# pierrebarbera/epa-ng

Measured on AMD Instinct MI355X. Metric: query placements/sec (whole node), 512-tip GTR+G4 DNA ref, preplace+thorough, higher is better.
Workload: dtype f64; 1 GPU; cfg2: 512-tip DNA GTR+G4 ref, W=1500, 150 bp reads, dyn-heur 0.99999, preplace+thorough; branches=1021, parallelism=query-shard x1 (weak)

## Files before the change

epa_ng_amd/csrc/epa_dev.hip:

```cpp
#include "epa_dev_internal.hpp"

#include <math.h>
#include <string.h>

#include <algorithm>
#include <numeric>
#include <atomic>
#include <thread>

static thread_local std::string g_create_err;

int epa_fail(epa_ctx* ctx, int code, const std::string& msg) {
  if (ctx) ctx->err = msg; else g_create_err = msg;
  return code;
}

namespace {
__global__ void __launch_bounds__(256) k_zero(uint4* __restrict__ a, size_t na, uint4* __restrict__ b, size_t nb) {
  const size_t stride = (size_t)gridDim.x * 256, i0 = (size_t)blockIdx.x * 256 + threadIdx.x;
  const uint4 z = make_uint4(0u, 0u, 0u, 0u);
  for (size_t i = i0; i < na; i += stride) a[i] = z;
  for (size_t i = i0; i < nb; i += stride) b[i] = z;
}
}
// ... 422 lines not shown
    if (code[t] != EPA_OK) { if (bad_query) *bad_query = bad[t]; return code[t]; }
  return EPA_OK;
}

extern "C" int epa_encode_queries(uint32_t states, uint32_t sites, uint32_t Q,
                                  const char* const* seqs, int premasking, int aa_x_as_n,
                                  uint8_t* codes, uint32_t* win_begin, uint32_t* win_span,
                                  uint32_t* bad_query) {
  return encode_impl(states, sites, Q, seqs, premasking, aa_x_as_n, false, 0, codes, win_begin, win_span,
                     bad_query);
}

extern "C" int epa_encode_queries_compact(uint32_t states, uint32_t sites, uint32_t Q,
                                          const char* const* seqs, int premasking, int aa_x_as_n,
                                          uint32_t stride, uint8_t* codes, uint32_t* win_begin,
                                          uint32_t* win_span, uint32_t* bad_query) {
  if (stride && !codes) return EPA_ERR_INVALID_ARG;
  return encode_impl(states, sites, Q, seqs, premasking, aa_x_as_n, true, stride, codes, win_begin,
                     win_span, bad_query);
}

extern "C" int epa_dev_device_count(void) {
  int n = 0;
  if (hipGetDeviceCount(&n) != hipSuccess) { (void)hipGetLastError(); return 0; }
  return n;
}

extern "C" const char* epa_dev_last_error(const epa_ctx* ctx) {
  return ctx ? ctx->err.c_str() : g_create_err.c_str();
}

extern "C" int epa_dev_set_query_layout(epa_ctx* ctx, uint32_t code_stride) {
  if (!ctx) return EPA_ERR_INVALID_ARG;
  ctx->code_stride = code_stride;
  return EPA_OK;
}

extern "C" int epa_dev_set_option(epa_ctx* ctx, const char* key, int value) {
  if (!ctx || !key) return EPA_ERR_INVALID_ARG;
  if (strcmp(key, "lookup_block") == 0) {
    if (!ctx->lookup_blocks) return epa_fail(ctx, EPA_ERR_INVALID_ARG, "set_option: lookup_block needs a context in the blocked lookup layout");
    if (value <= 0 || (value & 63)) return epa_fail(ctx, EPA_ERR_INVALID_ARG, "set_option: lookup_block must be a positive multiple of 64");
    for (void* p : ctx->blk_buf)
      if (p) return epa_fail(ctx, EPA_ERR_INVALID_ARG, "set_option: lookup_block must be set before the first preplacement");
    ctx->lookup_block = (uint32_t)value;
    return EPA_OK;
  }
  struct Entry { const char* name; int EpaOptions::*field; };
  static const Entry table[] = {
      {"thorough_generic", &EpaOptions::thorough_generic}, {"preplace_generic", &EpaOptions::preplace_generic},
      {"select_full_rows", &EpaOptions::select_full_rows}, {"select_sort", &EpaOptions::select_sort},
      {"queued_thorough", &EpaOptions::queued_thorough},   {"xcd_balance", &EpaOptions::xcd_balance},
      {"aa_valu", &EpaOptions::aa_valu},                   {"timers", &EpaOptions::timers},
      {"newton_lds", &EpaOptions::newton_lds}};
  for (const Entry& e : table)
    if (strcmp(key, e.name) == 0) {
      ctx->opt.*e.field = value;
      ctx->generic_thorough = ctx->generic_native || ctx->opt.thorough_generic != 0;
      return EPA_OK;
    }
  return epa_fail(ctx, EPA_ERR_INVALID_ARG, std::string("set_option: unknown key '") + key + "'");
}

extern "C" int epa_dev_set_heuristic(epa_ctx* ctx, int mode, double param) {
  if (!ctx) return EPA_ERR_INVALID_ARG;
  if (mode < EPA_HEUR_DYNAMIC || mode > EPA_HEUR_BASEBALL)
    return epa_fail(ctx, EPA_ERR_INVALID_ARG, "set_heuristic: unknown mode");
  if (mode == EPA_HEUR_FIXED && !(param >= 0.0 && param <= 1.0))
    return epa_fail(ctx, EPA_ERR_INVALID_ARG, "set_heuristic: the fraction must lie in [0, 1]");
  ctx->heur_mode = mode;
  ctx->heur_param = param;
  return EPA_OK;
}

extern "C" int epa_dev_set_query_packing(epa_ctx* ctx, int bits) {
  if (!ctx) return EPA_ERR_INVALID_ARG;
  if (bits != 8 && bits != 4) return epa_fail(ctx, EPA_ERR_INVALID_ARG, "set_query_packing: 8 or 4 bits per code");
  if (bits == 4 && ctx->s != 4)
    return epa_fail(ctx, EPA_ERR_UNSUPPORTED, "set_query_packing: the 4-bit format holds nucleotide codes only");
  ctx->code_packed4 = bits == 4;
  return EPA_OK;
}

extern "C" int epa_pack_codes_4bit(const uint8_t* codes, uint32_t Q, uint32_t stride, uint8_t* packed) {
  if (!codes || !packed) return EPA_ERR_INVALID_ARG;
  const size_t ps = ((size_t)stride + 1) / 2;
  const unsigned cap = g_encode_threads.load(std::memory_order_relaxed);
  const unsigned hw = cap ? cap : std::max(1u, std::thread::hardware_concurrency());
  const unsigned nt = (unsigned)std::min<uint64_t>(std::min(hw, 32u), std::max<uint64_t>(1, (uint64_t)Q * stride >> 20));
  std::vector<int> bad(nt, 0);
  auto work = [&](unsigned t) {
    const uint32_t q0 = (uint32_t)((uint64_t)Q * t / nt), q1 = (uint32_t)((uint64_t)Q * (t + 1) / nt);
    unsigned over = 0;
    for (uint32_t q = q0; q < q1; ++q) {
      const uint8_t* r = codes + (size_t)q * stride;
      uint8_t* o = packed + (size_t)q * ps;
      for (uint32_t p = 0; p < stride / 2; ++p) {
        const uint8_t hi = r[2 * p], lo = r[2 * p + 1];
        over |= hi | lo;
        o[p] = (uint8_t)((hi << 4) | lo);
      }
      if (stride & 1) { const uint8_t hi = r[stride - 1]; over |= hi; o[ps - 1] = (uint8_t)(hi << 4); }
    }
    bad[t] = over > 15;
  };
  if (nt == 1) work(0);
  else {
// ... 1958 lines not shown
```

epa_ng_amd/csrc/epa_dev_internal.hpp:

```cpp
#pragma once

#include <hip/hip_runtime.h>
#include <stdint.h>

#include <string>
#include <vector>

#include "epa_dev.h"

#define EPA_MAX_STATES 20
#define EPA_MAX_CATS 16
#define EPA_MAX_COLS 24
#define EPA_GRID_Y 65535u

struct ModelDNA {
  double U[16];
  double Ui[16];
  double lam[4];
  double rate[16];
  double w[16];
  double pi[4];
  int ng;
};

// ... 58 lines not shown
  size_t d_unpacked_sz = 0;
  size_t codes_bytes = 0;
  uint32_t Q = 0, stride = 0;
  bool packed4 = false;
  epa_pair* d_pairs = nullptr;
  epa_result* d_res = nullptr;
  size_t cap = 0;
  void* h_out = nullptr;
  size_t h_out_sz = 0;
  unsigned long long* h_stats = nullptr;
  unsigned long long* d_stats = nullptr;
  hipEvent_t ev_up = nullptr, ev_done = nullptr, ev_down = nullptr, ev_base = nullptr;
  hipStream_t stream = nullptr;
  const epa_pair* out_pairs = nullptr;
  const epa_result* out_res = nullptr;
  uint64_t n = 0;
  int state = 0;
  SelectPending sel;
  uint32_t* h_sel = nullptr;
  const uint8_t* l_codes = nullptr;
  const uint32_t *l_begin = nullptr, *l_span = nullptr;
  epa_pair* l_pairs = nullptr;
  epa_result* l_res = nullptr;
  uint32_t l_max_span = 0, l_flags = 0;
  int leader = -1;
  int g_index = 0;
  int g_n = 0;
  int g_left = 0;
  int g_slots[8] = {};
  uint32_t g_qoff[9] = {};
  uint32_t own_Q = 0;
  const uint8_t* own_x_codes = nullptr;
  const uint32_t *own_x_begin = nullptr, *own_x_span = nullptr;
  void* d_merge = nullptr;
  size_t d_merge_sz = 0;
  epa_pair* d_gpairs = nullptr;
  epa_result* d_gres = nullptr;
  size_t g_cap = 0;
  uint32_t* d_goff = nullptr;
  uint32_t* h_goff = nullptr;
};
constexpr int EPA_MAX_GROUP = 8;

struct EpaOptions {
  int thorough_generic = 0;
  int preplace_generic = 0;
  int select_full_rows = 0;
  int select_sort = 0;
  int queued_thorough = 0;
  int xcd_balance = 1;
  int aa_valu = 0;
  int timers = 1;
  int newton_lds = 0;
};

struct epa_ctx {
  int device = 0;
  EpaOptions opt;
  int n_cu = 256;
  hipStream_t stream = nullptr;
  std::string err;

  int s = 0, c = 0, ncols = 0;
  int c_in = 0;
  uint32_t W = 0, B = 0;
  ModelDev hmodel;
  ModelDev* dmodel = nullptr;
  ModelDNA dna;
  bool dna_zero0 = false;
  bool rate_scalers = false;
  bool generic_thorough = false;
  bool generic_native = false;
  BloConsts blo;
  int aa_x_as_n = 0;
  uint32_t code_stride = 0;

  double* refT = nullptr;
  uint32_t* scSum = nullptr;
  double* blen = nullptr;
  double* lookup = nullptr;
  double* refI = nullptr;
  uint8_t* resc0 = nullptr;
  double* cinv = nullptr;
  double inv_w0 = 0.0;
  double* lookup2 = nullptr;
  bool lookup_built = false;
  bool lookup_blocks = false;
  uint32_t lookup_block = 1024;
  std::vector<double> h_blen;

  static constexpr int N_SCRATCH = 18;
  static constexpr int N_SLOTS = 24;
  static constexpr int N_BANKS = 1 + N_SLOTS;
  int bank = 0;
  void* scratch[N_BANKS * N_SCRATCH] = {};
  size_t scratch_sz[N_BANKS * N_SCRATCH] = {};

  uint32_t* d_status = nullptr;
  uint32_t select_cap = 64;
  uint32_t* th_ctr = nullptr;
  uint32_t lnl_pitch = 0;
  unsigned long long* segmax = nullptr;
  uint32_t segp = 0;
  size_t segmax_zero_bytes = 0;
  bool code_packed4 = false;
  int heur_mode = 0;
// ... 107 lines not shown
```

epa_ng_amd/csrc/thorough_dna.hip:

```cpp
#include "epa_dev_internal.hpp"
#include "wave_util.hpp"

#include <cstring>
#include <rocprim/device/device_radix_sort.hpp>

using epa_radix_cfg = rocprim::radix_sort_config<rocprim::default_config, rocprim::default_config,
                                                 rocprim::default_config, 0>;

#include <algorithm>
#include <vector>
#include <cstdio>
#include <type_traits>
#include <cstdlib>

namespace {


struct ThArgs {
  ModelDNA m;
  BloConsts blo;
  const double* refT;
  const double* refI;
  const uint8_t* resc0;
  const double* cinv;
  double inv_w0;
  const uint32_t* scSum;
  const double* blen;
  const double* qt;
  const epa_pair* pairs;
  const uint32_t* order;
  const uint8_t* codes;
  uint32_t cstride, crel;
  const uint32_t* win_begin;
  const uint32_t* win_span;
  epa_result* out;
  unsigned long long* stats;
  uint32_t* qctr;
  double* sscratch;
  uint64_t n_pairs;
  uint32_t W;
  uint32_t Wpad;
  const uint32_t* spec;
  uint32_t spec_cls, spec_max;
  uint32_t xcum[9];
  uint32_t xstamp;
};

using namespace epa_wave;

__device__ __forceinline__ uint32_t zero_after(double v) {
  uint32_t z;
  asm volatile("v_mov_b32 %0, 0" : "=v"(z) : "v"(__double2loint(v)));
  return z;
}

using KArgs = const __attribute__((address_space(4))) ThArgs*;
__device__ __forceinline__ KArgs kargs_fresh() {
  KArgs p = (KArgs)__builtin_amdgcn_kernarg_segment_ptr();
  asm volatile("" : "+s"(p));
  return p;
}
struct PhaseModel {
  double U[16], Ui[16], w[4];
  __device__ __forceinline__ void load(uint32_t grp) {
    KArgs p = kargs_fresh();
#pragma unroll
    for (int i = 0; i < 16; ++i) { U[i] = p->m.U[i]; Ui[i] = p->m.Ui[i]; }
#pragma unroll
    for (int i = 0; i < 4; ++i) w[i] = p->m.w[grp * 4 + i];
  }
};

struct LaneConst {
  double lr;
  double cN;
  double w;
  int slot;
  int npos;
  const double* e2t;
  double lrn;
  double cn[3];
};

template <int N, class F>
__device__ __forceinline__ void static_for(F&& f) {
  if constexpr (N > 0) {
    static_for<N - 1>(f);
    f(std::integral_constant<int, N - 1>{});
  }
}
constexpr int dpp_pos(int k, int x) { return (k >> 1) * 8 + (k & 1) * 3 + x - 1; }
template <int N>
__device__ __forceinline__ void fmac_bcast(double& acc, double t, double s) {
  asm("v_fmac_f64_dpp %0, %1, %2 row_newbcast:%3 row_mask:0xf bank_mask:0xf" : "+v"(acc) : "v"(t), "v"(s), "i"(N));
}
__device__ __forceinline__ void dpp_ready(double& a, double& b, double& c) {
  asm("s_nop 1" : "+v"(a), "+v"(b), "+v"(c));
}
// ... 442 lines not shown
#pragma unroll
  for (int ch = 0; ch < NCH; ++ch) {
    double l0 = lsite[ch];
    bool mine = st.valid[ch];
    if (TAILH && ch == NCH - 1) mine = mine && lane < 32;
    if (!mine) l0 = 1.0;
    const int sc = mine ? (int)(st.sc[ch] + st.resc[ch]) : 0;
    mant *= __builtin_amdgcn_frexp_mant(l0);
    ex += __builtin_amdgcn_frexp_exp(l0) - 256 * sc;
    if ((ch & 7) == 7) {
      ex += __builtin_amdgcn_frexp_exp(mant);
      mant = __builtin_amdgcn_frexp_mant(mant);
    }
  }
  double v = wave_sum(log(mant) + (double)ex * 0.6931471805599453094), z = 0.0;
  cb.sum2(v, z, lane);
  return v;
}

template <int NCH, bool ZERO0, int NW, bool TAILH = false, int NG = 1, bool TDPP = false>
__device__ __forceinline__ double newton(const SiteState<NCH>& st, double* tab, int lane,
                                         const LaneConst& lc, Comb<NW, NG>& cb, double x1, double xguess,
                                         double x2, double tol, int max_iters, uint32_t& evals) {
  double rts = xguess, f, df, xl, xh, dx;
  if (rts < x1) rts = x1;
  if (rts > x2) rts = x2;
  derivatives<NCH, ZERO0, NW, TAILH, NG, TDPP>(st, tab, lane, lc, cb, rts, f, df);
  ++evals;
  if (!isfinite(f) || !isfinite(df)) return NAN;
  if (df >= 0.0 && fabs(f) < tol) return rts;
  if (f < 0.0) { xl = rts; xh = x2; } else { xh = rts; xl = x1; }
  for (int i = 1; i <= max_iters; ++i) {
    if (df <= 0.0 || (((rts - xh) * df - f) * ((rts - xl) * df - f) >= 0.0)) {
      dx = 0.5 * (xh - xl);
      rts = xl + dx;
      if (xl == rts) return rts;
    } else {
      dx = f / df;
      const double temp = rts;
      rts -= dx;
      if (temp == rts) return rts;
    }
    if (fabs(dx) < tol || i == max_iters) return rts;
    if (rts < x1) rts = x1;
    derivatives<NCH, ZERO0, NW, TAILH, NG, TDPP>(st, tab, lane, lc, cb, rts, f, df);
    ++evals;
    if (!isfinite(f) || !isfinite(df)) return NAN;
    if (df > 0.0 && fabs(f) < tol) return rts;
    if (f < 0.0) xl = rts; else xh = rts;
  }
  return NAN;
}

template <int NCH, bool ZERO0, bool INV, int NW, bool LOCAL, bool TAILH = false, int NG = 1, bool TDPP = false>
__device__ __forceinline__ void process_pair(const ThArgs& a, const uint64_t pidx, const int lane,
                                             double* tab, const double* qts, double* qa, const LaneConst& lc,
                                             Comb<NW, NG>& cb, uint32_t (&wstat)[3]) {
  static_assert(NG == 1 || NW == 1, "category groups and site blocks do not combine");
  const uint32_t site0 = NW > 1 ? (uint32_t)cb.wv * NCH * 64 : 0u;
  const uint32_t grp = NG > 1 ? (uint32_t)cb.wv : 0u;
  const uint64_t pid = a.order ? a.order[pidx] : pidx;
  const epa_pair pr = a.pairs[pid];
  const uint32_t b = (uint32_t)__builtin_amdgcn_readfirstlane((int)pr.branch_id);
  const uint32_t q = (uint32_t)__builtin_amdgcn_readfirstlane((int)pr.seq_id);
  const uint32_t begin = (uint32_t)__builtin_amdgcn_readfirstlane((int)a.win_begin[q]);
  const uint32_t n = (uint32_t)__builtin_amdgcn_readfirstlane((int)a.win_span[q]);
  const size_t cW = a.W;
  const char* ref = reinterpret_cast<const char*>(a.refT + ((size_t)(2 * b) * NG + grp) * 16 * cW + begin);
  const uint32_t W8 = a.W * 8u;
  const uint32_t* scp = a.scSum + (size_t)b * cW + begin;
  const uint8_t* qc = a.codes + (size_t)q * a.cstride + (a.crel ? 0u : begin);
  const double orig = a.blen[b];

  SiteState<NCH> st;
  const uint32_t half = TAILH ? (uint32_t)lane >> 5 : 0u;
  const uint32_t hoff = half * 8u * W8;
  double* const tabh = tab + (half << 3);
  auto lane_site = [&](int ch) -> uint32_t {
    return site0 + ch * 64 + ((TAILH && ch == NCH - 1) ? (uint32_t)lane & 31u : (uint32_t)lane);
  };
#pragma unroll
  for (int ch = 0; ch < NCH; ++ch) {
    const uint32_t s = lane_site(ch);
    st.valid[ch] = (NW == 1 && ch < NCH - 1) ? true : s < n;
    const uint32_t sc = st.valid[ch] ? s : 0;
    st.sc[ch] = scp[sc];
    st.code[ch] = qc[sc];
    st.resc[ch] = 0;
  }

  double tp = a.blo.pendant_default, td = orig * 0.5, tx = orig * 0.5;
  uint32_t evals = 0, rounds = 0, reverted = 0;
  uint32_t chain = 0;

  auto cinv_of = [&](int ch) -> double {
    const uint32_t s = st.valid[ch] ? lane_site(ch) : 0;
    const double v = a.cinv[begin + s] * a.inv_w0;
    if (NG > 1 && grp != 0) return 0.0;
    return (TAILH && ch == NCH - 1 && half) ? 0.0 : v;
  };
  const char* refi_s = reinterpret_cast<const char*>(a.refI + ((size_t)b * NG + grp) * 16 * cW + begin);
  auto stream_phase = [&](auto mode_c) {
    constexpr int MODE = decltype(mode_c)::value;
    constexpr int DEPTH = TH_STREAM_DEPTH;
    constexpr int NKL = TAILH ? 2 : 4;
    constexpr int NS = 4 * (NCH - 1) + NKL;
    constexpr int R = DEPTH + 1;
    PhaseModel pm;
    pm.load(grp);
    uint32_t W8p = W8;
    asm volatile("" : "+s"(W8p));
    double An[R][4], Bn[R][4];
    uint32_t soff[NCH], sidx[NCH];
#pragma unroll
    for (int ch = 0; ch < NCH; ++ch) {
      sidx[ch] = st.valid[ch] ? lane_site(ch) : 0;
      soff[ch] = sidx[ch] * 8u + ((TAILH && ch == NCH - 1) ? hoff : 0u);
    }
    uint32_t tok = chain;
    if constexpr (MODE == 1 || MODE == 3) {
      const int kq = lane & 3;
      const double* qv = qts + (lane >> 2) * 4;
      const double* e0 = tab + kq * 4;
      double av[4];
#pragma unroll
      for (int x = 0; x < 4; ++x) av[x] = qv[x] * e0[x];
      double* dst = qa + (lane >> 2) * QA_STRIDE + kq * 4;
#pragma unroll
      for (int i = 0; i < 4; ++i) {
        double v = pm.U[i * 4] * av[0];
#pragma unroll
        for (int x = 1; x < 4; ++x) v = fma(pm.U[i * 4 + x], av[x], v);
        dst[i] = v;
      }
      __builtin_amdgcn_fence(__ATOMIC_RELEASE, "wavefront");
      __builtin_amdgcn_wave_barrier();
      __builtin_amdgcn_fence(__ATOMIC_ACQUIRE, "wavefront");
    }
    auto issue = [&](int stp, uint32_t tk) {
      const int ch = stp >> 2, k = stp & 3, sl = stp % R;
      const uint32_t s0 = soff[ch] + tk;
#pragma unroll
      for (int x = 0; x < 4; ++x) {
        if (MODE == 2) An[sl][x] = *reinterpret_cast<const double*>(refi_s + (s0 + (uint32_t)(k * 4 + x) * W8p));
        else {
          An[sl][x] = *reinterpret_cast<const double*>(ref + (s0 + (uint32_t)(16 * NG + k * 4 + x) * W8p));
          Bn[sl][x] = *reinterpret_cast<const double*>(ref + (s0 + (uint32_t)(k * 4 + x) * W8p));
        }
      }
    };
#pragma unroll
    for (int p = 0; p < DEPTH; ++p)
      if (p < NS) issue(p, tok);
    int mx = 0;
    double qf[4];
#pragma unroll
    for (int stp = 0; stp < NS; ++stp) {
      const int ch = stp >> 2, k = stp & 3, sl = stp % R;
      const bool halfc = TAILH && ch == NCH - 1;
      const int NK = halfc ? 2 : 4;
      const double* tb = halfc ? tabh : tab;
      if (k == 0) {
        const double* qv = qts + st.code[ch] * 4;
        qf[0] = qv[0]; qf[1] = qv[1]; qf[2] = qv[2]; qf[3] = qv[3];
      }
      if (stp + DEPTH < NS) issue(stp + DEPTH, tok);
      asm volatile("" ::: "memory");
      double It[4];
      if (MODE == 2) {
#pragma unroll
        for (int x = 0; x < 4; ++x) It[x] = An[sl][x];
      } else if (MODE == 0) {
        cat_inner(pm, An[sl], tb + k * 4 + 2 * tok, Bn[sl], tb + 16 + k * 4 + 2 * tok, It, mx);
      } else {
        const double* ap = qa + st.code[ch] * QA_STRIDE + ((halfc ? (int)half * 2 : 0) + k) * 4 + 2 * tok;
        double Ap[4];
        lds_pair(ap, Ap[0], Ap[1]); lds_pair(ap + 2, Ap[2], Ap[3]);
        cat_inner_pre(pm, Ap, MODE == 1 ? Bn[sl] : An[sl], tb + 16 + k * 4 + 2 * tok, It, mx);
      }
#pragma unroll
      for (int x = 0; x < 4; ++x)
        st.S[ch][k * 4 + x] = It[x] * ((MODE == 0 || MODE == 2) ? qf[x] : (MODE == 1 ? An[sl][x] : Bn[sl][x]));
      tok = zero_after(st.S[ch][k * 4 + 3]);
      if (k == NK - 1) {
        if (MODE == 2) {
          st.resc[ch] = (a.resc0 + (size_t)b * cW + begin)[sidx[ch]];
        } else {
          int mxs = mx;
          if (halfc) {
            const auto sw = __builtin_amdgcn_permlane32_swap(mx, mx, false, false);
            mxs = max((int)sw[0], (int)sw[1]);
          }
          if constexpr (NG > 1) {
            double mv[1] = {(double)mxs};
            cb.template groups<1, true>(mv, lane);
            mxs = (int)mv[0];
          }
          const uint32_t resc = (mxs < 0x2ff00000) ? 1u : 0u;
          if (__builtin_amdgcn_ballot_w64(resc != 0) != 0) {
            const double mult = resc ? 0x1p+256 : 1.0;
#pragma unroll
            for (int i = 0; i < 16; ++i)
              if (i < NK * 4) st.S[ch][i] *= mult;
          }
          if (MODE == 0) st.resc[ch] = resc;
          mx = 0;
        }
        if constexpr (INV) st.S[ch][0] += cinv_of(ch);
        if constexpr (ZERO0) {
          if (halfc) st.S[ch][0] = fma(half ? pm.w[3] : pm.w[1], st.S[ch][4], (half ? pm.w[2] : pm.w[0]) * st.S[ch][0]);
          else st.S[ch][0] = fma(pm.w[3], st.S[ch][12], fma(pm.w[2], st.S[ch][8], fma(pm.w[1], st.S[ch][4], pm.w[0] * st.S[ch][0])));
        }
        tok = zero_after(st.S[ch][halfc ? 7 : 15]);
      }
    }
    chain = tok;
  };
  auto product_phase = [&](auto mode_c) { stream_phase(mode_c); };
  auto window_score = [&]() -> double {
    double ew[16];
#pragma unroll
    for (int i = 0; i < 8; ++i) lds_pair(tab + 32 + 2 * i, ew[2 * i], ew[2 * i + 1]);
    return window_lnl<NCH, ZERO0, NW, TAILH, NG>(st, ew, cb, lane, tab);
  };
  auto score = [&](double td_, double tx_, double tp_) -> double {
    const double tl = lc.slot == 0 ? td_ : (lc.slot == 1 ? tx_ : tp_);
    table_publish(tab, lane, TH_EXP(lc.lr * tl) * (lc.slot == 2 ? lc.w : 1.0));
    product_phase(std::integral_constant<int, 0>{});
    return window_score();
  };
  auto side_sumtable = [&](double tp_, double tother_, auto toward_prox) {
    constexpr bool TOWARD_PROX = decltype(toward_prox)::value;
    table_publish(tab, lane, TH_EXP(lc.lr * (lc.slot == 0 ? tp_ : tother_)));
    product_phase(std::integral_constant<int, TOWARD_PROX ? 3 : 1>{});
  };
  auto distal_sumtable = [&](double tp_, double tx_) { side_sumtable(tp_, tx_, std::false_type{}); };

  auto score_first = [&](double tp_) -> double {
    table_publish(tab, lane, TH_EXP(lc.lr * tp_) * (lc.slot == 2 ? lc.w : 1.0));
    stream_phase(std::integral_constant<int, 2>{});
    return window_score();
  };

  double loglikelihood = a.refI ? -score_first(tp) : -score(td, tx, tp);

  uint32_t smoothings = a.blo.max_rounds;
  if constexpr (LOCAL) {
    const double xmin = a.blo.min_branch, xmax = a.blo.max_branch, xtol = xmin / 10.0;
    auto solve = [&](double cur) -> double {
      double g = cur;
      if (g < xmin || g > xmax) g = a.blo.default_branch;
      const double r = newton<NCH, ZERO0, NW, TAILH, NG, TDPP>(st, tab, lane, lc, cb, xmin, g, xmax, xtol, (int)a.blo.max_newton, evals);
      chain = zero_after(r);
      return (isfinite(r) && fabs(cur - r) > 1e-10) ? r : cur;
    };
    while (smoothings) {
      tp = solve(tp);
      side_sumtable(tp, tx, std::false_type{});
      td = solve(td);
      side_sumtable(tp, td, std::true_type{});
      tx = solve(tx);
      (void)score(td, tx, tp);
      tp = solve(tp);
      table_publish(tab, lane, TH_EXP(lc.lr * tp) * (lc.slot == 2 ? lc.w : 1.0));
      double ew[16];
#pragma unroll
      for (int i = 0; i < 8; ++i) lds_pair(tab + 32 + 2 * i, ew[2 * i], ew[2 * i + 1]);
      const double new_ll = -window_lnl<NCH, ZERO0, NW, TAILH, NG>(st, ew, cb, lane, tab);
      ++rounds;
      --smoothings;
      if (fabs(new_ll - loglikelihood) < a.blo.epsilon) smoothings = 0;
      loglikelihood = new_ll;
    }
  }
  while (!LOCAL && smoothings) {
    const double old_td = td, old_tp = tp;
    double xmin = a.blo.min_branch, xmax = a.blo.max_branch, xtol = xmin / 10.0;
    double xguess = tp;
    if (xguess < xmin || xguess > xmax) xguess = a.blo.default_branch;
    double xres = newton<NCH, ZERO0, NW, TAILH, NG, TDPP>(st, tab, lane, lc, cb, xmin, xguess, xmax, xtol, (int)a.blo.max_newton, evals);
    if (xres > 0.0) tp = xres;
    chain = zero_after(tp);
    distal_sumtable(tp, tx);
    xguess = td;
    xmin = fmin(a.blo.min_branch / 2.0, orig / 2.0);
    xtol = xmin / 10.0;
    xmax = orig - xtol;
    if (xguess < xmin || xguess > xmax) xguess = orig / 2.0;
    xres = newton<NCH, ZERO0, NW, TAILH, NG, TDPP>(st, tab, lane, lc, cb, xmin, xguess, xmax, xtol, (int)a.blo.max_newton, evals);
    if (xres > 0.0) { td = xres; tx = orig - xres; }
    chain = zero_after(td);
    const double new_ll = -score(td, tx, tp);
    ++rounds;
    if (new_ll - loglikelihood > new_ll * 1e-14) {
      tp = old_tp; td = old_td; tx = orig - old_td;
      reverted = 1;
      break;
    }
    --smoothings;
    if (fabs(new_ll - loglikelihood) < a.blo.epsilon) smoothings = 0;
    loglikelihood = new_ll;
  }

  if (lane == 0 && ((NW == 1 && NG == 1) || cb.wv == 0)) {
    const double lnl = -loglikelihood;
    epa_result r;
    r.lnl = lnl;
    r.pendant_length = tp;
    r.distal_length = (orig / (td + tx)) * td;
    a.out[pid] = r;
    if (!isfinite(lnl)) {
      if (atomicAdd(&a.stats[3], 1ull) == 0) a.stats[4] = ((unsigned long long)b << 32) | q;
    }
  }
  wstat[0] += rounds;
  wstat[1] += evals;
  wstat[2] += reverted;
}

template <int NCH, bool ZERO0, bool INV, int NW, bool LOCAL = false, bool TAILH = false, int NG = 1, bool TDPP = false>
__global__ void __launch_bounds__(64 * NW * NG, TH_WAVES) k_thorough_dna(const ThArgs a) {
  constexpr int NWV = NW * NG;
  __shared__ __attribute__((aligned(16))) double tab[64 * NWV];
  __shared__ __attribute__((aligned(16))) double qts[64];
  __shared__ double red[2 * NW * 2];
  __shared__ double e2t[64];
  __shared__ __attribute__((aligned(16))) double qa[(16 * QA_STRIDE) * NWV];
  __shared__ double xch[NG > 1 ? 2 * NG * Comb<NW, NG>::XCH_MAX * 64 : 1];
  const int lane = threadIdx.x & 63;
  Comb<NW, NG> cb{red, (int)(threadIdx.x >> 6), 0, xch, 0};
  if (threadIdx.x < 64) {
    qts[lane] = a.qt[lane];
    e2t[lane] = exp2((double)lane * 0.015625);
  }
  LaneConst lc;
  lc.e2t = e2t;
  {
    const int lk = (lane >> 2) & 3, lx = lane & 3;
    const int kg = (NG > 1 ? cb.wv * 4 : 0) + lk;
    lc.slot = lane >> 4;
    lc.lr = a.m.lam[lx] * a.m.rate[kg];
    lc.w = a.m.w[kg];
    lc.cN = lc.slot == 0 ? lc.w : (lc.slot == 1 ? lc.w * lc.lr : (lc.slot == 2 ? lc.w * lc.lr * lc.lr : 0.0));
    const int dump = lc.slot == 3 ? 36 + (lane & 15) : 52 + lc.slot * 4 + lk;
    lc.npos = (lc.slot < 3 && lx != 0) ? lc.slot * 12 + lk * 3 + lx - 1 : dump;
  }
  if constexpr (TDPP) {
    const int p = lane & 15, q = p & 7;
    const int kn = q < 6 ? 2 * (p >> 3) + q / 3 : 0, xn = q % 3 + 1;
    const double wn = q < 6 ? a.m.w[kn] : 0.0;
    lc.lrn = q < 6 ? a.m.lam[xn] * a.m.rate[kn] : 0.0;
    lc.cn[0] = wn;
    lc.cn[1] = wn * lc.lrn;
    lc.cn[2] = wn * lc.lrn * lc.lrn;
  }
  __syncthreads();
  const uint32_t x = blockIdx.x & 7;
  const uint32_t w = blockIdx.x >> 3, stride = gridDim.x >> 3;
  uint64_t n_pairs = a.n_pairs;
  if constexpr (NW == 1 && NG == 1) {
    if (a.spec) {
      const uint32_t n = a.spec[0];
      if (n > a.spec_max || a.spec[9 + a.spec_cls] != n || a.spec[32] || a.spec[33]) return;
      n_pairs = n;
    }
  }
  const uint64_t per = (n_pairs + 7) / 8;
  uint64_t lo = (uint64_t)x * per;
  uint64_t hi = lo + per < n_pairs ? lo + per : n_pairs;
  if constexpr (NW == 1 && NG == 1) {
    lo = (n_pairs * a.xcum[x]) >> 20;
    hi = (n_pairs * a.xcum[x + 1]) >> 20;
    if (a.xstamp && blockIdx.x == 0 && threadIdx.x == 0) a.stats[7] = __builtin_amdgcn_s_memrealtime() & EPA_XSTAMP_MASK;
  }
  const unsigned long long clk0 = __builtin_amdgcn_s_memtime(), rt0 = __builtin_amdgcn_s_memrealtime();
  uint32_t wstat[3] = {0, 0, 0};
  if constexpr (NW == 1 && NG == 1) {
    uint32_t* ctr = a.qctr + x;
    const uint32_t cnt = (uint32_t)(hi > lo ? hi - lo : 0);
    uint32_t nxt = 0;
#ifdef TH_TIMING
    unsigned long long* tlog = reinterpret_cast<unsigned long long*>(a.sscratch) + (size_t)blockIdx.x * 8;
    unsigned long long t_first = 0, t_second = 0;
    uint32_t npr = 0;
    if (lane == 0) tlog[0] = __builtin_amdgcn_s_memrealtime();
#endif
    if (lane == 0) nxt = atomicAdd(ctr, 1u);
    nxt = (uint32_t)__builtin_amdgcn_readfirstlane((int)nxt);
    while (nxt < cnt) {
      const uint32_t cur = nxt;
      uint32_t f = 0;
      if (lane == 0) f = atomicAdd(ctr, 1u);
      process_pair<NCH, ZERO0, INV, NW, LOCAL, TAILH, NG, TDPP>(a, lo + cur, lane, tab + cb.wv * 64, qts, qa + cb.wv * (16 * QA_STRIDE), lc, cb, wstat);
      nxt = (uint32_t)__builtin_amdgcn_readfirstlane((int)f);
#ifdef TH_TIMING
      ++npr;
      if (npr == 1) t_first = __builtin_amdgcn_s_memrealtime();
      if (npr == 2) t_second = __builtin_amdgcn_s_memrealtime();
#endif
    }
#ifdef TH_TIMING
    if (lane == 0) { tlog[1] = t_first; tlog[2] = t_second; tlog[3] = __builtin_amdgcn_s_memrealtime(); tlog[4] = npr; }
#endif
  } else {
    for (uint64_t p = lo + w; p < hi; p += stride)
      process_pair<NCH, ZERO0, INV, NW, LOCAL, TAILH, NG, TDPP>(a, p, lane, tab + cb.wv * 64, qts, qa + cb.wv * (16 * QA_STRIDE), lc, cb, wstat);
  }
  if (threadIdx.x == 0) {
    atomicAdd(&a.stats[0], (unsigned long long)wstat[0]);
    atomicAdd(&a.stats[1], (unsigned long long)wstat[1]);
    atomicAdd(&a.stats[2], (unsigned long long)wstat[2]);
    if constexpr (NW == 1 && NG == 1) {
      if (a.xstamp) atomicMax(&a.stats[8 + x], ((unsigned long long)(__builtin_amdgcn_s_memrealtime() & EPA_XSTAMP_MASK) << 21) |
                                                   (unsigned long long)(a.xcum[x + 1] - a.xcum[x]));
    }
    if (a.xstamp && blockIdx.x == 0) {
      a.stats[5] = __builtin_amdgcn_s_memtime() - clk0;
      a.stats[6] = __builtin_amdgcn_s_memrealtime() - rt0;
    }
  }
}

#ifdef TH_ONLY_MAIN
template __global__ void k_thorough_dna<3, true, false, 1, false, true, 1>(const ThArgs a);
template __global__ void k_thorough_dna<3, true, false, 1, false, true, 1, true>(const ThArgs a);
}
#else
template <class Deriv>
__device__ __forceinline__ double newton_fn(Deriv&& deriv, double x1, double xguess, double x2, double tol,
                                            int max_iters, uint32_t& evals) {
  double rts = xguess, f, df, xl, xh, dx;
  if (rts < x1) rts = x1;
  if (rts > x2) rts = x2;
  deriv(rts, f, df);
  ++evals;
  if (!isfinite(f) || !isfinite(df)) return NAN;
  if (df >= 0.0 && fabs(f) < tol) return rts;
  if (f < 0.0) { xl = rts; xh = x2; } else { xh = rts; xl = x1; }
  for (int i = 1; i <= max_iters; ++i) {
    if (df <= 0.0 || (((rts - xh) * df - f) * ((rts - xl) * df - f) >= 0.0)) {
      dx = 0.5 * (xh - xl);
      rts = xl + dx;
      if (xl == rts) return rts;
    } else {
      dx = f / df;
      const double temp = rts;
      rts -= dx;
      if (temp == rts) return rts;
    }
    if (fabs(dx) < tol || i == max_iters) return rts;
    if (rts < x1) rts = x1;
    deriv(rts, f, df);
    ++evals;
    if (!isfinite(f) || !isfinite(df)) return NAN;
    if (df > 0.0 && fabs(f) < tol) return rts;
    if (f < 0.0) xl = rts; else xh = rts;
  }
  return NAN;
}
// ... 274 lines not shown
#undef LAUNCH_GN
#undef LAUNCH_G
    return EPA_OK;
  }
  const bool tailh = cls == 10 || cls == 11;
  constexpr bool n4_off = false;
  switch (cls) {
    case 0: LAUNCH(1, 1); break;
    case 1: case 10: LAUNCH(2, 1); break;
    case 2: case 11: LAUNCH(3, 1); break;
    case 3: if (n4_off) LAUNCH(2, 2); else LAUNCH(4, 1); break;
    case 4: LAUNCH(3, 2); break;
    case 5: LAUNCH(2, 4); break;
    case 6: LAUNCH(3, 4); break;
    case 7: LAUNCH(2, 8); break;
    case 8: LAUNCH(3, 8); break;
    default: {
      const uint32_t nlong = (uint32_t)std::min<uint64_t>(n_pairs, 2048);
      a.Wpad = (max_span + 63) / 64 * 64;
      a.sscratch = (double*)epa_scratch(ctx, 7, sizeof(double) * (size_t)nlong * 17 * a.Wpad);
      if (!a.sscratch) return epa_fail(ctx, EPA_ERR_HIP, "hipMalloc(long-window sumtable scratch)");
      if (ctx->dna_zero0) hipLaunchKernelGGL((k_thorough_dna_long<true>), dim3(nlong), dim3(64), 0, ctx->stream, a);
      else hipLaunchKernelGGL((k_thorough_dna_long<false>), dim3(nlong), dim3(64), 0, ctx->stream, a);
    }
  }
#undef LAUNCH
#ifdef TH_TIMING
  if (a.sscratch && (cls <= 2 || cls == 10 || cls == 11)) {
    std::vector<unsigned long long> h(2048 * 8);
    (void)hipStreamSynchronize(ctx->stream);
    (void)hipMemcpy(h.data(), a.sscratch, 2048 * 64, hipMemcpyDeviceToHost);
    unsigned long long t0 = ~0ull, t1 = 0;
    for (int w = 0; w < 2048; ++w) if (h[w * 8]) { t0 = std::min(t0, h[w * 8]); t1 = std::max(t1, h[w * 8 + 3]); }
    std::vector<double> st, fp, sp, ex, np_;
    for (int w = 0; w < 2048; ++w) {
      if (!h[w * 8]) continue;
      st.push_back((h[w * 8] - t0) * 0.01);
      if (h[w * 8 + 1]) fp.push_back((h[w * 8 + 1] - h[w * 8]) * 0.01);
      if (h[w * 8 + 2]) sp.push_back((h[w * 8 + 2] - h[w * 8 + 1]) * 0.01);
      ex.push_back((h[w * 8 + 3] - t0) * 0.01);
      np_.push_back((double)h[w * 8 + 4]);
    }
    for (int x = 0; x < 8; ++x) {
      double e0 = 1e30, e1 = 0, fsum = 0; unsigned long long np2 = 0; int nw = 0;
      for (int w = x; w < 2048; w += 8) {
        if (!h[w * 8]) continue;
        const double e = (h[w * 8 + 3] - t0) * 0.01;
        e0 = std::min(e0, e); e1 = std::max(e1, e); np2 += h[w * 8 + 4]; ++nw;
        if (h[w * 8 + 1]) fsum += (h[w * 8 + 1] - h[w * 8]) * 0.01;
      }
      fprintf(stderr, "  x %d: waves %d pairs %llu exit %.1f .. %.1f us, mean first pair %.1f\n", x, nw, np2, e0, e1, nw ? fsum / nw : 0.0);
    }
    auto pct = [](std::vector<double>& v, double p) { if (v.empty()) return 0.0; std::sort(v.begin(), v.end()); return v[(size_t)(p * (v.size() - 1))]; };
    fprintf(stderr, "TH_TIMING n_pairs %llu: span %.1f us | wave start p50 %.1f p99 %.1f max %.1f | first pair p50 %.1f p90 %.1f max %.1f | second pair p50 %.1f p90 %.1f | exit p1 %.1f p10 %.1f p50 %.1f p90 %.1f max %.1f | pairs/wave p50 %.0f max %.0f\n",
            (unsigned long long)a.n_pairs, (t1 - t0) * 0.01, pct(st, 0.5), pct(st, 0.99), pct(st, 1.0), pct(fp, 0.5), pct(fp, 0.9), pct(fp, 1.0), pct(sp, 0.5), pct(sp, 0.9),
            pct(ex, 0.01), pct(ex, 0.1), pct(ex, 0.5), pct(ex, 0.9), pct(ex, 1.0), pct(np_, 0.5), pct(np_, 1.0));
  }
#endif
  return EPA_OK;
}

static ThArgs dna_args(epa_ctx* ctx, const epa_pair* d_pairs, const uint32_t* ord, const uint8_t* d_codes,
                       const uint32_t* d_begin, const uint32_t* d_span, epa_result* d_out, unsigned long long* d_stats) {
  ThArgs a;
  a.m = ctx->dna;
  a.blo = ctx->blo;
  a.refT = ctx->refT;
  a.refI = ctx->lookup_built ? ctx->refI : nullptr;
  a.resc0 = ctx->resc0;
  a.cinv = ctx->cinv;
  a.inv_w0 = ctx->inv_w0;
  a.scSum = ctx->scSum;
  a.blen = ctx->blen;
  a.qt = ctx->dmodel->qt;
  a.pairs = d_pairs;
  a.order = ord;
  a.codes = d_codes;
  a.crel = ctx->code_stride ? 1u : 0u;
  a.cstride = a.crel ? ctx->code_stride : ctx->W;
  a.win_begin = d_begin;
  a.win_span = d_span;
  a.out = d_out;
  a.stats = d_stats;
  a.sscratch = nullptr;
  a.qctr = nullptr;
  a.n_pairs = 0;
  a.W = ctx->W;
  a.Wpad = 0;
  a.spec = nullptr;
  a.spec_cls = 0;
  a.spec_max = 0;
  for (int i = 0; i < 9; ++i) a.xcum[i] = ctx->xcd_cum[i];
  a.xstamp = 0;
  return a;
}

int launch_thorough_queued(epa_ctx* ctx, const epa_pair* d_pairs, const uint32_t* d_spec, uint64_t max_pairs,
                           const uint8_t* d_codes, const uint32_t* d_begin, const uint32_t* d_span, uint32_t max_span,
                           epa_result* d_out, unsigned long long* d_stats) {
  if (ctx->s != 4 || ctx->generic_thorough || ctx->dna.ng != 1 || !epa_th_ctr(ctx) || !d_span || !d_spec) return -1;
  if (max_pairs > 0xffffffffull) return -1;
  const int cls = epa_span_class(4, max_span);
  if (!(cls <= 2 || cls == 10 || cls == 11)) return -1;
  static const uint32_t bound[12] = {64, 128, 192, 0, 0, 0, 0, 0, 0, 0, 96, 160};
  ThArgs a = dna_args(ctx, d_pairs, nullptr, d_codes, d_begin, d_span, d_out, d_stats);
  a.n_pairs = 0xffffffffull;
  a.spec = d_spec;
  a.spec_cls = (uint32_t)cls;
  a.spec_max = (uint32_t)max_pairs;
  a.xstamp = 1u;
  epa_timer_start(ctx, epa_t(ctx, epa_ctx::T_THOROUGH));
  const int rc = launch_thorough_dna_class(ctx, a, cls, std::min(max_span, bound[cls]));
  epa_timer_stop(ctx, epa_t(ctx, epa_ctx::T_THOROUGH));
  if (rc) return -2;
  if (hipGetLastError() != hipSuccess) { (void)epa_fail(ctx, EPA_ERR_HIP, "queued thorough launch"); return -2; }
  return cls;
}

int launch_thorough(epa_ctx* ctx, const epa_pair* d_pairs, uint64_t n_pairs, const uint8_t* d_codes,
                    const uint32_t* d_begin, const uint32_t* d_span, uint32_t max_span,
                    epa_result* d_out, unsigned long long* d_stats, const uint32_t* cls_hist) {
  if (n_pairs > 0xffffffffull) return epa_fail(ctx, EPA_ERR_INVALID_ARG, "thorough: more than 2^32 pairs per call");
  if (ctx->generic_thorough || (!ctx->blo.sliding && ctx->s == 4 && max_span > 1536u)) {
    return launch_thorough_generic(ctx, d_pairs, n_pairs, d_codes, d_begin, d_span, max_span, d_out, d_stats);
  }
  uint32_t hist[EPA_N_CLS] = {};
  const int cmax = epa_span_class(ctx->s, max_span);
  uint64_t given = 0;
  if (cls_hist) for (int c = 0; c < EPA_N_CLS; ++c) given += cls_hist[c];
  const bool cached = cls_hist && given == n_pairs && n_pairs != 0;
  if (cached) {
    for (int c = 0; c < EPA_N_CLS; ++c) hist[c] = cls_hist[c];
  } else if (cmax == 0) {
    hist[0] = (uint32_t)n_pairs;
  }
  size_t temp_bytes = 0;
  (void)rocprim::radix_sort_pairs<epa_radix_cfg>(nullptr, temp_bytes, (uint32_t*)nullptr, (uint32_t*)nullptr,
                                  (uint32_t*)nullptr, (uint32_t*)nullptr, (size_t)n_pairs, 0, 4, ctx->stream);
  const size_t nb = (sizeof(uint32_t) * n_pairs + 255) & ~(size_t)255;
  uint32_t* d_hist = nullptr;
  uint32_t *d_keys = nullptr, *d_idx = nullptr, *d_keys2 = nullptr, *d_order = nullptr;
  auto carve = [&]() -> int {
    char* base = (char*)epa_scratch(ctx, 8, 256 + 4 * nb + temp_bytes);
    if (!base) return epa_fail(ctx, EPA_ERR_HIP, "hipMalloc(span-class scratch)");
    d_hist = (uint32_t*)base;
    d_keys = (uint32_t*)(base + 256); d_idx = (uint32_t*)(base + 256 + nb);
// ... 65 lines not shown
```

Baseline: 16.83 million placements/s.

## Prefetch next thorough pair's metadata and site data during current Newton iterations

In the dynamic-queue thorough DNA kernel, each wave now loads the next pair's index, branch/query ids, window bounds, branch length and per-lane scaler sums and query codes in stages spread across the current pair's Newton and sumtable steps. The next call then takes these values from carried registers instead of starting with a chain of dependent global loads. This is meant to hide the pointer-chasing latency at the start of each pair. It costs extra live registers, which may reduce occupancy, and it applies only to some template configurations. A new pair_prefetch option, on by default, controls it, and a profiling script is added.

New measurement: 16.78 million placements/s. Within noise of the previous version (-0.3%).

```diff
diff --git a/epa_ng_amd/csrc/epa_dev.hip b/epa_ng_amd/csrc/epa_dev.hip
--- a/epa_ng_amd/csrc/epa_dev.hip
+++ b/epa_ng_amd/csrc/epa_dev.hip
@@ -498,7 +498,7 @@
       {"select_full_rows", &EpaOptions::select_full_rows}, {"select_sort", &EpaOptions::select_sort},
       {"queued_thorough", &EpaOptions::queued_thorough},   {"xcd_balance", &EpaOptions::xcd_balance},
       {"aa_valu", &EpaOptions::aa_valu},                   {"timers", &EpaOptions::timers},
-      {"newton_lds", &EpaOptions::newton_lds}};
+      {"newton_lds", &EpaOptions::newton_lds},             {"pair_prefetch", &EpaOptions::pair_prefetch}};
   for (const Entry& e : table)
     if (strcmp(key, e.name) == 0) {
       ctx->opt.*e.field = value;
diff --git a/epa_ng_amd/csrc/epa_dev_internal.hpp b/epa_ng_amd/csrc/epa_dev_internal.hpp
--- a/epa_ng_amd/csrc/epa_dev_internal.hpp
+++ b/epa_ng_amd/csrc/epa_dev_internal.hpp
@@ -134,6 +134,7 @@
   int aa_valu = 0;
   int timers = 1;
   int newton_lds = 0;
+  int pair_prefetch = 1;
 };
 
 struct epa_ctx {
diff --git a/epa_ng_amd/csrc/thorough_dna.hip b/epa_ng_amd/csrc/thorough_dna.hip
--- a/epa_ng_amd/csrc/thorough_dna.hip
+++ b/epa_ng_amd/csrc/thorough_dna.hip
@@ -44,6 +44,7 @@
   uint32_t spec_cls, spec_max;
   uint32_t xcum[9];
   uint32_t xstamp;
+  uint32_t pair_prefetch;
 };
 
 using namespace epa_wave;
@@ -592,42 +593,122 @@
   return NAN;
 }
 
+template <int NCH>
+struct PairCarry {
+  uint32_t have = 0;
+  uint32_t pid;
+  uint32_t bq;
+  uint32_t win;
+  uint32_t sc[NCH], code[NCH];
+  uint64_t lo = 0;
+  uint32_t cnt = 0, f = 0;
+#ifdef TH_TIMING
+  unsigned long long tsum[3] = {0, 0, 0};
+  unsigned long long t0 = 0;
+#endif
+};
+__device__ __forceinline__ uint32_t lane_of(uint32_t v, int l) { return (uint32_t)__builtin_amdgcn_readlane((int)v, l); }
+
 template <int NCH, bool ZERO0, bool INV, int NW, bool LOCAL, bool TAILH = false, int NG = 1, bool TDPP = false>
 __device__ __forceinline__ void process_pair(const ThArgs& a, const uint64_t pidx, const int lane,
                                              double* tab, const double* qts, double* qa, const LaneConst& lc,
-                                             Comb<NW, NG>& cb, uint32_t (&wstat)[3]) {
+                                             Comb<NW, NG>& cb, uint32_t (&wstat)[3], PairCarry<NCH>& pc) {
   static_assert(NG == 1 || NW == 1, "category groups and site blocks do not combine");
+  constexpr bool CARRY = NW == 1 && NG == 1 && !LOCAL && (NCH <= 2 || (NCH == 3 && ZERO0 && !INV));
+  constexpr bool AHEAD = CARRY;
   const uint32_t site0 = NW > 1 ? (uint32_t)cb.wv * NCH * 64 : 0u;
   const uint32_t grp = NG > 1 ? (uint32_t)cb.wv : 0u;
-  const uint64_t pid = a.order ? a.order[pidx] : pidx;
-  const epa_pair pr = a.pairs[pid];
-  const uint32_t b = (uint32_t)__builtin_amdgcn_readfirstlane((int)pr.branch_id);
-  const uint32_t q = (uint32_t)__builtin_amdgcn_readfirstlane((int)pr.seq_id);
-  const uint32_t begin = (uint32_t)__builtin_amdgcn_readfirstlane((int)a.win_begin[q]);
-  const uint32_t n = (uint32_t)__builtin_amdgcn_readfirstlane((int)a.win_span[q]);
   const size_t cW = a.W;
+  auto lane_site = [&](int ch) -> uint32_t {
+    return site0 + ch * 64 + ((TAILH && ch == NCH - 1) ? (uint32_t)lane & 31u : (uint32_t)lane);
+  };
+  auto link_pid = [&](uint64_t at, uint32_t vz) {
+    pc.pid = a.order ? a.order[at + vz] : (uint32_t)at + vz;
+  };
+  auto link_pair = [&]() {
+    pc.bq = reinterpret_cast<const uint32_t*>(a.pairs)[(size_t)pc.pid * 2 + ((uint32_t)lane & 1u)];
+  };
+  auto link_win = [&]() {
+    const uint32_t nb = lane_of(pc.bq, 0), nq = lane_of(pc.bq, 1);
+    const uint32_t l3 = (uint32_t)lane & 3u;
+    const uint32_t* pb = reinterpret_cast<const uint32_t*>(a.blen + nb) + (l3 & 1u);
+    const uint32_t* pw = (l3 & 1u) ? a.win_span + nq : a.win_begin + nq;
+    pc.win = *((l3 & 2u) ? pb : pw);
+  };
+  auto link_lanes = [&]() {
+    const uint32_t nb = lane_of(pc.bq, 0), nq = lane_of(pc.bq, 1);
+    const uint32_t nbegin = lane_of(pc.win, 0), nn = lane_of(pc.win, 1);
+    const uint32_t* scp = a.scSum + (size_t)nb * cW + nbegin;
+    const uint8_t* qc = a.codes + (size_t)nq * a.cstride + (a.crel ? 0u : nbegin);
+#pragma unroll
+    for (int ch = 0; ch < NCH; ++ch) {
+      const uint32_t s = lane_site(ch);
+      const uint32_t sc = (ch < NCH - 1 || s < nn) ? s : 0;
+      pc.sc[ch] = scp[sc];
+      pc.code[ch] = qc[sc];
+    }
+  };
+  uint64_t pid;
+  uint32_t b, q, begin, n;
+  double orig;
+  if constexpr (CARRY) {
+#ifdef TH_TIMING
+    pc.t0 = __builtin_amdgcn_s_memtime();
+#endif
+    if (!pc.have) {
+      uint32_t vz;
+      asm volatile("v_mov_b32 %0, 0" : "=v"(vz));
+      link_pid(pidx, vz);
+      link_pair();
+      link_win();
+      link_lanes();
+    }
+    pc.have = 0;
+    pid = lane_of(pc.pid, 0);
+    b = lane_of(pc.bq, 0);
+    q = lane_of(pc.bq, 1);
+    begin = lane_of(pc.win, 0);
+    n = lane_of(pc.win, 1);
+    orig = __hiloint2double((int)lane_of(pc.win, 3), (int)lane_of(pc.win, 2));
+  } else {
+    pid = a.order ? a.order[pidx] : pidx;
+    const epa_pair pr = a.pairs[pid];
+    b = (uint32_t)__builtin_amdgcn_readfirstlane((int)pr.branch_id);
+    q = (uint32_t)__builtin_amdgcn_readfirstlane((int)pr.seq_id);
+    begin = (uint32_t)__builtin_amdgcn_readfirstlane((int)a.win_begin[q]);
+    n = (uint32_t)__builtin_amdgcn_readfirstlane((int)a.win_span[q]);
+    orig = a.blen[b];
+  }
   const char* ref = reinterpret_cast<const char*>(a.refT + ((size_t)(2 * b) * NG + grp) * 16 * cW + begin);
   const uint32_t W8 = a.W * 8u;
-  const uint32_t* scp = a.scSum + (size_t)b * cW + begin;
-  const uint8_t* qc = a.codes + (size_t)q * a.cstride + (a.crel ? 0u : begin);
-  const double orig = a.blen[b];
 
   SiteState<NCH> st;
   const uint32_t half = TAILH ? (uint32_t)lane >> 5 : 0u;
   const uint32_t hoff = half * 8u * W8;
   double* const tabh = tab + (half << 3);
-  auto lane_site = [&](int ch) -> uint32_t {
-    return site0 + ch * 64 + ((TAILH && ch == NCH - 1) ? (uint32_t)lane & 31u : (uint32_t)lane);
-  };
 #pragma unroll
   for (int ch = 0; ch < NCH; ++ch) {
     const uint32_t s = lane_site(ch);
     st.valid[ch] = (NW == 1 && ch < NCH - 1) ? true : s < n;
-    const uint32_t sc = st.valid[ch] ? s : 0;
-    st.sc[ch] = scp[sc];
-    st.code[ch] = qc[sc];
+    if constexpr (CARRY) {
+      st.sc[ch] = pc.sc[ch];
+      st.code[ch] = pc.code[ch];
+    } else {
+      const uint32_t* scp = a.scSum + (size_t)b * cW + begin;
+      const uint8_t* qc = a.codes + (size_t)q * a.cstride + (a.crel ? 0u : begin);
+      const uint32_t sc = st.valid[ch] ? s : 0;
+      st.sc[ch] = scp[sc];
+      st.code[ch] = qc[sc];
+    }
     st.resc[ch] = 0;
   }
+#ifdef TH_TIMING
+  if constexpr (CARRY) {
+#pragma unroll
+    for (int ch = 0; ch < NCH; ++ch) asm volatile("" ::"v"(st.sc[ch]), "v"(st.code[ch]));
+    pc.tsum[0] += __builtin_amdgcn_s_memtime() - pc.t0;
+  }
+#endif
 
   double tp = a.blo.pendant_default, td = orig * 0.5, tx = orig * 0.5;
   uint32_t evals = 0, rounds = 0, reverted = 0;
@@ -722,6 +803,10 @@
       for (int x = 0; x < 4; ++x)
         st.S[ch][k * 4 + x] = It[x] * ((MODE == 0 || MODE == 2) ? qf[x] : (MODE == 1 ? An[sl][x] : Bn[sl][x]));
       tok = zero_after(st.S[ch][k * 4 + 3]);
+#ifdef TH_TIMING
+      if constexpr (CARRY && MODE == 2)
+        if (stp == 0) pc.tsum[1] += __builtin_amdgcn_s_memtime() - pc.t0;
+#endif
       if (k == NK - 1) {
         if (MODE == 2) {
           st.resc[ch] = (a.resc0 + (size_t)b * cW + begin)[sidx[ch]];
@@ -783,6 +868,11 @@
   };
 
   double loglikelihood = a.refI ? -score_first(tp) : -score(td, tx, tp);
+  if constexpr (AHEAD) {
+    const uint32_t fn = min((uint32_t)__builtin_amdgcn_readfirstlane((int)pc.f), pc.cnt - 1u);
+    link_pid(pc.lo + fn, zero_after(loglikelihood));
+    asm volatile("" ::: "memory");
+  }
 
   uint32_t smoothings = a.blo.max_rounds;
   if constexpr (LOCAL) {
@@ -821,7 +911,9 @@
     double xres = newton<NCH, ZERO0, NW, TAILH, NG, TDPP>(st, tab, lane, lc, cb, xmin, xguess, xmax, xtol, (int)a.blo.max_newton, evals);
     if (xres > 0.0) tp = xres;
     chain = zero_after(tp);
+    if constexpr (AHEAD) { link_pair(); asm volatile("" ::: "memory"); }
     distal_sumtable(tp, tx);
+    if constexpr (AHEAD) { link_win(); asm volatile("" ::: "memory"); }
     xguess = td;
     xmin = fmin(a.blo.min_branch / 2.0, orig / 2.0);
     xtol = xmin / 10.0;
@@ -830,6 +922,11 @@
     xres = newton<NCH, ZERO0, NW, TAILH, NG, TDPP>(st, tab, lane, lc, cb, xmin, xguess, xmax, xtol, (int)a.blo.max_newton, evals);
     if (xres > 0.0) { td = xres; tx = orig - xres; }
     chain = zero_after(td);
+    if constexpr (AHEAD) {
+      link_lanes();
+      asm volatile("" ::: "memory");
+      pc.have = a.pair_prefetch;
+    }
     const double new_ll = -score(td, tx, tp);
     ++rounds;
     if (new_ll - loglikelihood > new_ll * 1e-14) {
@@ -856,6 +953,9 @@
   wstat[0] += rounds;
   wstat[1] += evals;
   wstat[2] += reverted;
+#ifdef TH_TIMING
+  if constexpr (CARRY) pc.tsum[2] += __builtin_amdgcn_s_memtime() - pc.t0;
+#endif
 }
 
 template <int NCH, bool ZERO0, bool INV, int NW, bool LOCAL = false, bool TAILH = false, int NG = 1, bool TDPP = false>
@@ -915,10 +1015,13 @@
   }
   const unsigned long long clk0 = __builtin_amdgcn_s_memtime(), rt0 = __builtin_amdgcn_s_memrealtime();
   uint32_t wstat[3] = {0, 0, 0};
+  PairCarry<NCH> pc;
   if constexpr (NW == 1 && NG == 1) {
     uint32_t* ctr = a.qctr + x;
     const uint32_t cnt = (uint32_t)(hi > lo ? hi - lo : 0);
     uint32_t nxt = 0;
+    pc.lo = lo;
+    pc.cnt = cnt;
 #ifdef TH_TIMING
     unsigned long long* tlog = reinterpret_cast<unsigned long long*>(a.sscratch) + (size_t)blockIdx.x * 8;
     unsigned long long t_first = 0, t_second = 0;
@@ -929,10 +1032,10 @@
     nxt = (uint32_t)__builtin_amdgcn_readfirstlane((int)nxt);
     while (nxt < cnt) {
       const uint32_t cur = nxt;
-      uint32_t f = 0;
-      if (lane == 0) f = atomicAdd(ctr, 1u);
-      process_pair<NCH, ZERO0, INV, NW, LOCAL, TAILH, NG, TDPP>(a, lo + cur, lane, tab + cb.wv * 64, qts, qa + cb.wv * (16 * QA_STRIDE), lc, cb, wstat);
-      nxt = (uint32_t)__builtin_amdgcn_readfirstlane((int)f);
+      pc.f = 0;
+      if (lane == 0) pc.f = atomicAdd(ctr, 1u);
+      process_pair<NCH, ZERO0, INV, NW, LOCAL, TAILH, NG, TDPP>(a, lo + cur, lane, tab + cb.wv * 64, qts, qa + cb.wv * (16 * QA_STRIDE), lc, cb, wstat, pc);
+      nxt = (uint32_t)__builtin_amdgcn_readfirstlane((int)pc.f);
 #ifdef TH_TIMING
       ++npr;
       if (npr == 1) t_first = __builtin_amdgcn_s_memrealtime();
@@ -940,11 +1043,14 @@
 #endif
     }
 #ifdef TH_TIMING
-    if (lane == 0) { tlog[1] = t_first; tlog[2] = t_second; tlog[3] = __builtin_amdgcn_s_memrealtime(); tlog[4] = npr; }
+    if (lane == 0) {
+      tlog[1] = t_first; tlog[2] = t_second; tlog[3] = __builtin_amdgcn_s_memrealtime(); tlog[4] = npr;
+      tlog[5] = pc.tsum[0]; tlog[6] = pc.tsum[1]; tlog[7] = pc.tsum[2];
+    }
 #endif
   } else {
     for (uint64_t p = lo + w; p < hi; p += stride)
-      process_pair<NCH, ZERO0, INV, NW, LOCAL, TAILH, NG, TDPP>(a, p, lane, tab + cb.wv * 64, qts, qa + cb.wv * (16 * QA_STRIDE), lc, cb, wstat);
+      process_pair<NCH, ZERO0, INV, NW, LOCAL, TAILH, NG, TDPP>(a, p, lane, tab + cb.wv * 64, qts, qa + cb.wv * (16 * QA_STRIDE), lc, cb, wstat, pc);
   }
   if (threadIdx.x == 0) {
     atomicAdd(&a.stats[0], (unsigned long long)wstat[0]);
@@ -1325,6 +1431,15 @@
       fprintf(stderr, "  x %d: waves %d pairs %llu exit %.1f .. %.1f us, mean first pair %.1f\n", x, nw, np2, e0, e1, nw ? fsum / nw : 0.0);
     }
     auto pct = [](std::vector<double>& v, double p) { if (v.empty()) return 0.0; std::sort(v.begin(), v.end()); return v[(size_t)(p * (v.size() - 1))]; };
+    std::vector<double> pa, pb, pp, sa, sb;
+    for (int w = 0; w < 2048; ++w) {
+      if (!h[w * 8] || !h[w * 8 + 4] || !h[w * 8 + 7]) continue;
+      const double np1 = (double)h[w * 8 + 4], tot = (double)h[w * 8 + 7];
+      pa.push_back(h[w * 8 + 5] / np1); pb.push_back(h[w * 8 + 6] / np1); pp.push_back(tot / np1);
+      sa.push_back(100.0 * h[w * 8 + 5] / tot); sb.push_back(100.0 * h[w * 8 + 6] / tot);
+    }
+    fprintf(stderr, "TH_TIMING prologue (pair_prefetch %u): cycles per pair to registers p50 %.0f p90 %.0f | to first product p50 %.0f p90 %.0f | pair p50 %.0f p90 %.0f | share of the pair, to registers p50 %.2f %% p90 %.2f %% | to first product p50 %.2f %% p90 %.2f %%\n",
+            a.pair_prefetch, pct(pa, 0.5), pct(pa, 0.9), pct(pb, 0.5), pct(pb, 0.9), pct(pp, 0.5), pct(pp, 0.9), pct(sa, 0.5), pct(sa, 0.9), pct(sb, 0.5), pct(sb, 0.9));
     fprintf(stderr, "TH_TIMING n_pairs %llu: span %.1f us | wave start p50 %.1f p99 %.1f max %.1f | first pair p50 %.1f p90 %.1f max %.1f | second pair p50 %.1f p90 %.1f | exit p1 %.1f p10 %.1f p50 %.1f p90 %.1f max %.1f | pairs/wave p50 %.0f max %.0f\n",
             (unsigned long long)a.n_pairs, (t1 - t0) * 0.01, pct(st, 0.5), pct(st, 0.99), pct(st, 1.0), pct(fp, 0.5), pct(fp, 0.9), pct(fp, 1.0), pct(sp, 0.5), pct(sp, 0.9),
             pct(ex, 0.01), pct(ex, 0.1), pct(ex, 0.5), pct(ex, 0.9), pct(ex, 1.0), pct(np_, 0.5), pct(np_, 1.0));
@@ -1365,6 +1480,7 @@
   a.spec_max = 0;
   for (int i = 0; i < 9; ++i) a.xcum[i] = ctx->xcd_cum[i];
   a.xstamp = 0;
+  a.pair_prefetch = ctx->opt.pair_prefetch ? 1u : 0u;
   return a;
 }
 
diff --git a/profiles/pair_prologue.py b/profiles/pair_prologue.py
--- /dev/null
+++ b/profiles/pair_prologue.py
@@ -0,0 +1,42 @@
+#!/usr/bin/env python3
+import os
+import sys
+
+import numpy as np
+import torch
+
+sys.path.insert(0, os.path.dirname(os.path.dirname(os.path.abspath(__file__))))
+import epa_ng_amd as epa
+from epa_ng_amd import hostlib, synth
+
+root = synth.random_tree(512, 1)
+rates = synth.gamma_rates(synth.CFG2_ALPHA)
+labels, seqs = synth.simulate_msa(root, 1500, synth.CFG2_SUBST, synth.CFG2_FREQS, rates, 2)
+ref = hostlib.Reference(synth.newick(root), labels, seqs, states=4, subst=synth.CFG2_SUBST, freqs=synth.CFG2_FREQS,
+                        rates=rates)
+ev = ref.evaluator()
+codes, wb, ws = synth.make_reads_compact(seqs, 100000, 150, 0.03, 3, 4)
+dev = torch.device("cuda", 0)
+dc = torch.from_numpy(codes).to(dev)
+dwb, dws = torch.from_numpy(wb.view(np.int32)).to(dev), torch.from_numpy(ws.view(np.int32)).to(dev)
+cap = 100000 * 64
+dp = torch.empty((cap, 2), dtype=torch.int32, device=dev)
+dr = torch.zeros((cap, 3), dtype=torch.float64, device=dev)
+print("== the chunk body (its Newton launch is stamped too)", file=sys.stderr, flush=True)
+ev.chunk_stage(0, dc, dwb, dws)
+ev.chunk_launch(0, max_span=150, max_pairs=cap, pairs_out=dp, results_out=dr, keep_on_device=True)
+n = ev.chunk_finish_device(0)
+pairs = np.zeros(n, epa.PAIR_DTYPE)
+hp = dp[:n].cpu().numpy()
+pairs["branch_id"], pairs["seq_id"] = hp[:, 0], hp[:, 1]
+res = {}
+for prefetch in (0, 1, 0, 1, 0, 1):
+    print("== thorough alone, %d pairs, pair_prefetch %d" % (n, prefetch), file=sys.stderr, flush=True)
+    ev.set_option("pair_prefetch", prefetch)
+    r = ev.thorough(pairs, codes, wb, ws)
+    res.setdefault(prefetch, r.copy())
+    assert all(np.array_equal(r[f], res[prefetch][f]) for f in r.dtype.names)
+same = all(np.array_equal(res[0][f], res[1][f]) for f in res[0].dtype.names)
+print("== results of pair_prefetch 0 and 1 array_equal: %s; rounds per pair %.3f" % (same, ev.last_stats["rounds"] / n),
+      file=sys.stderr, flush=True)
+sys.exit(0 if same else 1)
```
